# filodb/FiloDB

Measured on NVIDIA H100. Metric: samples/s scanned+aggregated (rate over 10M series); % HBM roofline, higher is better.
Workload: dtype f64

## Files before the change

### filodb_b200/csrc/scan_kernels.cu

```cuda
#include <cuda_runtime.h>
#include <stdint.h>
#define FILO_DEV_ERR_TS_WIRE 1
#define FILO_DEV_ERR_VAL_WIRE 2
#define FILO_DEV_ERR_EMPTY 3
#define FILO_DEV_ERR_SCRATCH 4
#include "scan_device.cuh"
#include "kernels.h"
#include "scan_fast.cuh"
#include "scan_tile.cuh"
#include "scan_wp.cuh"
#include "scan_wp_ctr.cuh"

namespace filo {

__device__ __forceinline__ void report_error(int* d_err, int code, int64_t series) {
  if (atomicCAS(&d_err[0], 0, code) == 0) { d_err[1] = (int)(series & 0x7fffffff); d_err[2] = (int)(series >> 31); }
}

__device__ __forceinline__ int resolve_series(const uint8_t* rec, const QueryParams& q, uint8_t* scratch, uint32_t scratch_bytes,
                                              bool need_corrected, int lane, int& err, int64_t& rows_scanned, int64_t& bytes_scanned) {
  const RecordHeader* h = reinterpret_cast<const RecordHeader*>(rec);
  const ChunkEntry* E = reinterpret_cast<const ChunkEntry*>(rec + sizeof(RecordHeader));
  const int nch = (int)h->n_chunks;
  const int64_t t1 = q.start - q.window, t2 = q.end;
// ... 342 lines not shown
                   unsigned long long* d_counters, int* d_err,
                   const int64_t* __restrict__ list, const unsigned long long* __restrict__ list_count) {
  MomOnly<MOM, double*> pval2;
  if constexpr (MOM) pval2.v = pval + (size_t)n_items * q.T;
  if (list) n_items = (int64_t)*list_count;
  extern __shared__ __align__(128) uint8_t smem[];
  const int warp = threadIdx.x >> 5, lane = threadIdx.x & 31;
  const int64_t gw = (int64_t)blockIdx.x * FAST_WARPS + warp, nw = (int64_t)gridDim.x * FAST_WARPS;
  const uint32_t per_warp = WARP_HDR_BYTES + rec_cap + STAGE_BYTES + acc_bytes + scratch_bytes;
  uint8_t* base = smem + (size_t)warp * per_warp;
  WarpStage st{reinterpret_cast<uint64_t*>(base), base + WARP_HDR_BYTES, rec_cap, 0, false, arena, rec_off};
  double* stage = reinterpret_cast<double*>(base + WARP_HDR_BYTES + rec_cap);
  double* acc = reinterpret_cast<double*>(base + WARP_HDR_BYTES + rec_cap + STAGE_BYTES);
  MomOnly<MOM, double*> acc2;
  if constexpr (MOM) acc2.v = acc + q.T;
  uint32_t* cnt = reinterpret_cast<uint32_t*>(base + WARP_HDR_BYTES + rec_cap + STAGE_BYTES + (size_t)q.T * (MOM ? 16 : 8));
  uint8_t* scratch = base + WARP_HDR_BYTES + rec_cap + STAGE_BYTES + acc_bytes;
  if (lane == 0) { mbar_init(st.bar, 1); mbar_fence_init(); }
  __syncwarp();
  const double ident = agg_op == AGG_MIN ? __longlong_as_double(0x7ff0000000000000LL)
                     : agg_op == AGG_MAX ? __longlong_as_double(0xfff0000000000000LL) : 0.0;
  int64_t rows = 0, bytes = 0;
  int64_t it = gw;
  int64_t pos = 0, pend = 0;
  auto real_item = [&](int64_t x) -> int64_t { return list ? list[x] : x; };
  auto advance_item = [&]() { while (it < n_items) { const int64_t ri = real_item(it); pos = item_begin[ri]; pend = item_begin[ri + 1]; if (pos < pend) return true; it += nw; } return false; };
  bool have = advance_item();
  if (have) st.issue(order ? order[pos] : pos, lane);
  while (have) {
    for (int k = lane; k < q.T; k += 32) { acc[k] = ident; cnt[k] = 0; if constexpr (MOM) acc2.v[k] = 0.0; }
    __syncwarp();
    const int64_t my_item = real_item(it);
    while (true) {
      const int64_t i = order ? order[pos] : pos;
      int64_t npos = pos + 1, nit = it, npend = pend; bool nhave = true;
      if (npos >= pend) { nit = it + nw; nhave = false; while (nit < n_items) { const int64_t ri = real_item(nit); npos = item_begin[ri]; npend = item_begin[ri + 1]; if (npos < npend) { nhave = true; break; } nit += nw; } }
      const int64_t inext = nhave ? (order ? order[npos] : npos) : -1;
      const uint8_t* rec = st.acquire(i);
      int err;
      process_series<CLS>(rec, q, scratch, scratch_bytes, stage, lane, err, rows, bytes,
                     [&](int k, double v, bool valid) {
                       if (valid && v == v) {
                         double a = acc[k];
                         if (agg_op == AGG_MIN) a = a < v ? a : v;
                         else if (agg_op == AGG_MAX) a = a > v ? a : v;
                         else if (agg_op != AGG_COUNT) a += v;
                         acc[k] = a; cnt[k] += 1;
                         if constexpr (MOM) acc2.v[k] += v * v;
                       }
                     },
                     [&]() { if (inext >= 0) st.issue(inext, lane); });
      if (err) {
        if (lane == 0) report_error(d_err, err, i);
        __syncwarp();
        if (inext >= 0) st.issue(inext, lane);
      }
      __syncwarp();
      const bool same_item = nhave && nit == it;
      pos = npos; pend = npend; it = nit; have = nhave;
      if (!same_item) break;
    }
    double* pv = pval + (size_t)my_item * q.T; uint32_t* pc = pcnt + (size_t)my_item * q.T;
    for (int k = lane; k < q.T; k += 32) { pv[k] = acc[k]; pc[k] = cnt[k]; }
    if constexpr (MOM) { double* pv2 = pval2.v + (size_t)my_item * q.T; for (int k = lane; k < q.T; k += 32) pv2[k] = acc2.v[k]; }
    __syncwarp();
  }
  if (lane == 0 && (rows | bytes)) { atomicAdd(&d_counters[0], (unsigned long long)rows); atomicAdd(&d_counters[1], (unsigned long long)bytes); }
}

#ifndef FILO_CUSIM
#ifdef FILO_TILE_PROF
extern "C" int filo_debug_tile_prof(unsigned long long* out16, int reset) {
  cudaError_t e = cudaMemcpyFromSymbol(out16, g_tile_prof, sizeof(unsigned long long) * 16);
  if (e == cudaSuccess && reset) { unsigned long long z[16] = {}; e = cudaMemcpyToSymbol(g_tile_prof, z, sizeof z); }
  return (int)e;
}
#endif
#ifdef FILO_WP_PROF
extern "C" int filo_debug_wp_prof(unsigned long long* out32, int reset) {
  cudaError_t e = cudaMemcpyFromSymbol(out32, g_wp_prof, sizeof(unsigned long long) * 32);
  if (e == cudaSuccess && reset) { unsigned long long z[32] = {}; e = cudaMemcpyToSymbol(g_wp_prof, z, sizeof z); }
  return (int)e;
}
#endif
template <int CLS>
static cudaError_t launch_series_v2_cls(const ScanLaunch& L, double* out, uint32_t rec_cap, size_t smem) {
  cudaError_t e = cudaFuncSetAttribute(scan_series_kernel_v2<CLS>, cudaFuncAttributeMaxDynamicSharedMemorySize, (int)smem);
  if (e != cudaSuccess) return e;
  scan_series_kernel_v2<CLS><<<L.grid, FAST_WARPS * 32, smem, L.stream>>>(L.arena, L.rec_off, L.n_series, L.q, out, rec_cap, L.scratch_bytes,
                                                                           L.d_counters, L.d_err, L.list, L.list_count);
  return cudaGetLastError();
}
cudaError_t launch_scan_series_v2(const ScanLaunch& L, double* out, uint32_t rec_cap) {
  const size_t smem = (size_t)(WARP_HDR_BYTES + rec_cap + STAGE_BYTES + L.scratch_bytes) * FAST_WARPS;
  switch (fn_class_of(L.q.fn, L.q.cumulative, L.q.long_values)) {
    case CLASS_SUM: return launch_series_v2_cls<CLASS_SUM>(L, out, rec_cap, smem);
    case CLASS_MINMAX: return launch_series_v2_cls<CLASS_MINMAX>(L, out, rec_cap, smem);
    case CLASS_COUNTER: return launch_series_v2_cls<CLASS_COUNTER>(L, out, rec_cap, smem);
    default: return launch_series_v2_cls<CLASS_POINT>(L, out, rec_cap, smem);
  }
}
template <int CLS, bool MOM>
static cudaError_t launch_agg_v2_cls(const ScanLaunch& L, const int32_t* order, const int64_t* item_begin, int64_t n_items, int agg_op,
                                     double* pval, uint32_t* pcnt, uint32_t acc_bytes, uint32_t rec_cap, size_t smem) {
  cudaError_t e = cudaFuncSetAttribute(scan_agg_kernel_v2<CLS, MOM>, cudaFuncAttributeMaxDynamicSharedMemorySize, (int)smem);
  if (e != cudaSuccess) return e;
  scan_agg_kernel_v2<CLS, MOM><<<L.grid, FAST_WARPS * 32, smem, L.stream>>>(L.arena, L.rec_off, order, item_begin, n_items, L.q, agg_op, pval, pcnt,
                                                                             rec_cap, L.scratch_bytes, acc_bytes, L.d_counters, L.d_err, L.list, L.list_count);
  return cudaGetLastError();
}
template <bool MOM>
static cudaError_t launch_agg_v2_any(const ScanLaunch& L, const int32_t* order, const int64_t* item_begin, int64_t n_items, int agg_op,
                                     double* pval, uint32_t* pcnt, uint32_t acc_bytes, uint32_t rec_cap, size_t smem) {
  switch (fn_class_of(L.q.fn, L.q.cumulative, L.q.long_values)) {
    case CLASS_SUM: return launch_agg_v2_cls<CLASS_SUM, MOM>(L, order, item_begin, n_items, agg_op, pval, pcnt, acc_bytes, rec_cap, smem);
    case CLASS_MINMAX: return launch_agg_v2_cls<CLASS_MINMAX, MOM>(L, order, item_begin, n_items, agg_op, pval, pcnt, acc_bytes, rec_cap, smem);
    case CLASS_COUNTER: return launch_agg_v2_cls<CLASS_COUNTER, MOM>(L, order, item_begin, n_items, agg_op, pval, pcnt, acc_bytes, rec_cap, smem);
    default: return launch_agg_v2_cls<CLASS_POINT, MOM>(L, order, item_begin, n_items, agg_op, pval, pcnt, acc_bytes, rec_cap, smem);
  }
}
cudaError_t launch_scan_agg_v2(const ScanLaunch& L, const int32_t* order, const int64_t* item_begin, int64_t n_items, int agg_op,
                               double* pval, uint32_t* pcnt, uint32_t acc_bytes, uint32_t rec_cap, bool moments) {
  const size_t smem = (size_t)(WARP_HDR_BYTES + rec_cap + STAGE_BYTES + acc_bytes + L.scratch_bytes) * FAST_WARPS;
  return moments ? launch_agg_v2_any<true>(L, order, item_begin, n_items, agg_op, pval, pcnt, acc_bytes, rec_cap, smem)
                 : launch_agg_v2_any<false>(L, order, item_begin, n_items, agg_op, pval, pcnt, acc_bytes, rec_cap, smem);
}
struct TileAggArgs { const int32_t* order; const int64_t* item_begin; int64_t n_items; int agg_op; double* pval; uint32_t* pcnt; };
template <int FN, bool AGG, bool MOM>
static cudaError_t launch_tile_fn(const ScanLaunch& L, double* out, const TileSmem& T, int64_t* fallback_list, unsigned long long* fallback_count,
                                  const TileAggArgs& A) {
  cudaError_t e = cudaFuncSetAttribute(scan_tile_kernel<FN, AGG, MOM>, cudaFuncAttributeMaxDynamicSharedMemorySize, (int)T.total);
  if (e != cudaSuccess) return e;
  scan_tile_kernel<FN, AGG, MOM><<<L.grid, TILE_LAUNCH_THREADS, T.total, L.stream>>>(L.arena, L.rec_off, L.n_series, L.q, out, T, fallback_list, fallback_count,
      L.d_counters, L.d_err, A.order, A.item_begin, A.n_items, A.agg_op, A.pval, A.pcnt);
  return cudaGetLastError();
}
template <bool AGG, bool MOM = false>
static cudaError_t launch_tile_any(const ScanLaunch& L, double* out, const TileSmem& T, int64_t* fallback_list, unsigned long long* fallback_count,
                                   const TileAggArgs& A) {
  switch (L.q.fn) {
    case FN_RATE: return launch_tile_fn<FN_RATE, AGG, MOM>(L, out, T, fallback_list, fallback_count, A);
    case FN_AVG: return launch_tile_fn<FN_AVG, AGG, MOM>(L, out, T, fallback_list, fallback_count, A);
    case FN_COUNT: return launch_tile_fn<FN_COUNT, AGG, MOM>(L, out, T, fallback_list, fallback_count, A);
    default: return launch_tile_fn<FN_SUM, AGG, MOM>(L, out, T, fallback_list, fallback_count, A);
  }
}
cudaError_t launch_scan_tile(const ScanLaunch& L, double* out, const TileSmem& T, int64_t* fallback_list, unsigned long long* fallback_count) {
  return launch_tile_any<false>(L, out, T, fallback_list, fallback_count, TileAggArgs{nullptr, nullptr, 0, 0, nullptr, nullptr});
}
cudaError_t launch_scan_tile_agg(const ScanLaunch& L, const TileSmem& T, const int32_t* order, const int64_t* item_begin, int64_t n_items, int agg_op,
                                 double* pval, uint32_t* pcnt, int64_t* fallback_list, unsigned long long* fallback_count, bool moments) {
  const TileAggArgs A{order, item_begin, n_items, agg_op, pval, pcnt};
  return moments ? launch_tile_any<true, true>(L, nullptr, T, fallback_list, fallback_count, A)
                 : launch_tile_any<true>(L, nullptr, T, fallback_list, fallback_count, A);
}
template <int FN, int NW>
static cudaError_t launch_wp_nw(const ScanLaunch& L, double* out, const WpSmem& W, int64_t* fallback_list, unsigned long long* fallback_count) {
  const size_t smem = (size_t)W.per_warp * W.warps;
  cudaError_t e = cudaFuncSetAttribute(scan_wp_sum_kernel<FN, NW>, cudaFuncAttributeMaxDynamicSharedMemorySize, (int)smem);
  if (e != cudaSuccess) return e;
  scan_wp_sum_kernel<FN, NW><<<L.grid, W.warps * 32, smem, L.stream>>>(L.arena, L.rec_off, L.n_series, L.q, out, W, fallback_list, fallback_count, L.d_counters, L.d_err);
  return cudaGetLastError();
}
template <int FN>
static cudaError_t launch_wp_fn(const ScanLaunch& L, double* out, const WpSmem& W, int64_t* fallback_list, unsigned long long* fallback_count) {
  if (W.warps <= (uint32_t)WP_MAX_WARPS) return launch_wp_nw<FN, WP_MAX_WARPS>(L, out, W, fallback_list, fallback_count);
// ... 123 lines not shown
```

### filodb_b200/csrc/scan_wp_ctr.cuh

```cuda
#pragma once
#include "scan_wp.cuh"

namespace filo {

__device__ __forceinline__ double drops_cum(const TileDrops& D, int r) {
  const int n = D.n < TILE_MAXDROP ? D.n : TILE_MAXDROP;
  double cum = 0.0;
#pragma unroll
  for (int j = 0; j < TILE_MAXDROP; ++j) if (j < n && D.pos[j] <= r) cum = D.amt[j];
  return cum;
}

template <bool IS_COUNTER, bool IS_RATE>
__device__ __forceinline__ double extrapolated_rate_tile(int64_t windowStart, int64_t windowEnd, int32_t numSamples, int64_t t1, double v1,
                                                         int64_t t2, double v2, double fdiv, double frcp, int64_t step, const TileCtrTab* tab) {
  double durationToStart = div_invariant((double)(t1 - windowStart), 1000.0, 0.001);
  const double durationToEnd = div_invariant((double)(windowEnd - t2), 1000.0, 0.001);
  const int64_t si_ms = t2 - t1;
  const int m = numSamples - 1;
  double sampledInterval, extrapolationThreshold, half, rcpSI;
  if (m <= TILE_CTR_TABMAX && si_ms == (int64_t)m * step) {
    const TileCtrTab e = tab[m];
    sampledInterval = e.sI; extrapolationThreshold = e.thr; half = e.half; rcpSI = e.rcpSI;
  } else {
// ... 34 lines not shown
    if (ch.end_time < wStart) continue;
    if (c > 0 && !(K[c - 1].end_time < wEnd)) continue;
    int su = ch.s0 + k; if (su < 0) su = 0;
    int eu = ch.e0 + k; if (eu > ch.nrows - 1) eu = ch.nrows - 1;
    const double first = __longlong_as_double((long long)CD[c].first);
    if (FN != FN_DELTA && some) { if (first != first || first < corrLast) corr = corr + corrLast; }
    if (su <= eu) {
      const int64_t tS = ch.init + (int64_t)su * qstep, tE = ch.init + (int64_t)eu * qstep;
      const bool skip = FN != FN_DELTA && su == 0 && eu == 0 && first != first;
      if (!skip && (tS < loT || tE > hiT)) {
        numSamples += eu - su + 1;
        const bool drp = FN != FN_DELTA && ch.kc.dropped;
        if (tS < loT) { loT = tS; const double b = wp_ctr_value(V, ch, su, DR[c], drp); loV = (FN != FN_DELTA && some) ? b + corr : b; }
        if (tE > hiT) { hiT = tE; const double b = wp_ctr_value(V, ch, eu, DR[c], drp); hiV = (FN != FN_DELTA && some) ? b + corr : b; }
      }
    }
    if (FN != FN_DELTA) {
      if (ch.kc.dropped) {
        int idx = ch.nrows - 1; double lastValue = 0.0;
        do { lastValue = wp_row(V, ch, idx); idx -= 1; } while (lastValue != lastValue && idx >= 0);
        corrLast = nan0(lastValue); corr = (some ? corr : 0.0) + drops_cum(DR[c], ch.nrows - 1);
      }
      else { corrLast = wp_row(V, ch, ch.nrows - 1); corr = some ? corr : 0.0; }
    }
    some = true;
  }
  const int64_t cws = qinclusive ? wStart : wStart - 1;
  if (hiT > loT) return extrapolated_rate_tile<FN != FN_DELTA, FN == FN_RATE>(cws, wEnd, numSamples, loT, loV, hiT, hiV, fdiv, frcp, qstep, tab);
  return NaNv;
}

__device__ __forceinline__ int wp_irr_lower(const int32_t* TSR, const WpCtrChunk& ch, int64_t t) {
  const int64_t d64 = t - ch.init;
  if (d64 <= 0) return 0;
  const int32_t* p = TSR + ch.rowpos;
  const int nr = ch.nrows;
  if (d64 > (int64_t)p[nr - 1]) return nr;
  const int32_t d = (int32_t)d64;
  int g = (int)((float)d * __int_as_float(ch.kc.pad));
  if (g > nr - 1) g = nr - 1;
  while (g < nr && p[g] < d) ++g;
  while (g > 0 && p[g - 1] >= d) --g;
  return g;
}
template <int FN>
__device__ __forceinline__ double wp_eval_counter_irr(int n, const WpCtrChunk* K, const WpChunk* CD, const TileDrops* DR, const double* V, const int32_t* TSR,
                                                      int64_t qstep, int qinclusive, int64_t wStart, int64_t wEnd, double fdiv, double frcp, const TileCtrTab* tab) {
  const double NaNv = __longlong_as_double(0x7ff8000000000000LL);
  int32_t numSamples = 0; int64_t loT = INT64_MAX, hiT = 0; double loV = NaNv, hiV = NaNv;
  bool some = false; double corrLast = 0.0, corr = 0.0;
  for (int c = 0; c < n; ++c) {
    const WpCtrChunk& ch = K[c];
    if (ch.end_time < wStart) continue;
    if (c > 0 && !(K[c - 1].end_time < wEnd)) continue;
    const int su = wp_irr_lower(TSR, ch, wStart);
    int eu = wp_irr_lower(TSR, ch, wEnd + 1) - 1; if (eu > ch.nrows - 1) eu = ch.nrows - 1;
    const double first = __longlong_as_double((long long)CD[c].first);
    if (FN != FN_DELTA && some) { if (first != first || first < corrLast) corr = corr + corrLast; }
    if (su <= eu) {
      const int64_t tS = ch.init + (int64_t)TSR[ch.rowpos + su], tE = ch.init + (int64_t)TSR[ch.rowpos + eu];
      const bool skip = FN != FN_DELTA && su == 0 && eu == 0 && first != first;
      if (!skip && (tS < loT || tE > hiT)) {
        numSamples += eu - su + 1;
        const bool drp = FN != FN_DELTA && ch.kc.dropped;
        if (tS < loT) { loT = tS; const double b = wp_ctr_value(V, ch, su, DR[c], drp); loV = (FN != FN_DELTA && some) ? b + corr : b; }
        if (tE > hiT) { hiT = tE; const double b = wp_ctr_value(V, ch, eu, DR[c], drp); hiV = (FN != FN_DELTA && some) ? b + corr : b; }
      }
    }
    if (FN != FN_DELTA) {
      if (ch.kc.dropped) {
        int idx = ch.nrows - 1; double lastValue = 0.0;
        do { lastValue = wp_row(V, ch, idx); idx -= 1; } while (lastValue != lastValue && idx >= 0);
        corrLast = nan0(lastValue); corr = (some ? corr : 0.0) + drops_cum(DR[c], ch.nrows - 1);
      }
      else { corrLast = wp_row(V, ch, ch.nrows - 1); corr = some ? corr : 0.0; }
    }
    some = true;
  }
  const int64_t cws = qinclusive ? wStart : wStart - 1;
  if (hiT > loT) return extrapolated_rate_tile<FN != FN_DELTA, FN == FN_RATE>(cws, wEnd, numSamples, loT, loV, hiT, hiV, fdiv, frcp, qstep, tab);
  return NaNv;
}

#ifdef FILO_CUSIM
inline void wp_bump_u16(uint16_t* p) { *p = (uint16_t)(*p + 1); }
#else
static __device__ __noinline__ void wp_bump_u16(uint16_t* p) { *p = (uint16_t)(*p + 1); }
#endif
template <int FN>
__device__ __forceinline__ double wp_clamped_window(const double* V, const WpCtrChunk& ch, const TileDrops& D, bool drp, int kk, int64_t wEnd, int64_t cws, int64_t qstep,
                                                   double fdiv, double frcp, const TileCtrTab* tab) {
  int r1 = ch.s0 + kk; if (r1 < 0) r1 = 0;
  int r2 = ch.e0 + kk; if (r2 > ch.nrows - 1) r2 = ch.nrows - 1;
  if (!(r2 > r1)) return __longlong_as_double(0x7ff8000000000000LL);
  double v1 = wp_row(V, ch, r1), v2 = wp_row(V, ch, r2);
  if (drp) { v1 = nan0(v1) + drops_cum(D, r1); v2 = nan0(v2) + drops_cum(D, r2); }
  return extrapolated_rate_tile<FN != FN_DELTA, FN == FN_RATE>(cws, wEnd, r2 - r1 + 1, ch.init + (int64_t)r1 * qstep, v1, ch.init + (int64_t)r2 * qstep, v2,
                                                              fdiv, frcp, qstep, tab);
}

template <int FN, bool AGG, int NW, bool IRR = false, bool MOM = false>
__global__ void __launch_bounds__(NW * 32, 1)
scan_wp_ctr_kernel(const uint8_t* __restrict__ arena, const int64_t* __restrict__ rec_off, int64_t n_series, QueryParams q,
                   double* __restrict__ out, WpCtrSmem L, int64_t* __restrict__ fallback_list, unsigned long long* __restrict__ fallback_count,
                   unsigned long long* d_counters, int* d_err,
                   const int32_t* __restrict__ order, const int64_t* __restrict__ item_begin, int64_t n_items, int agg_op,
                   double* __restrict__ pval, uint32_t* __restrict__ pcnt) {
  extern __shared__ __align__(128) uint8_t smem[];
  const unsigned FULL = 0xffffffffu;
  const int lane = threadIdx.x & 31, warp = threadIdx.x >> 5;
  uint8_t* wb = smem + (size_t)warp * L.per_warp;
  uint64_t* bar = reinterpret_cast<uint64_t*>(wb);
  WpChunk* CD = reinterpret_cast<WpChunk*>(wb + WP_OFF_DESC);
  uint64_t* xtab = reinterpret_cast<uint64_t*>(wb + WP_OFF_J);
  TileDrops* DR = reinterpret_cast<TileDrops*>(wb + WP_OFF_DROPS);
  uint8_t* R = wb + WP_OFF_REC;
  double* V = reinterpret_cast<double*>(wb + L.vals);
  WpCtrChunk* KC = reinterpret_cast<WpCtrChunk*>(wb + L.kc);
  double* ACC = reinterpret_cast<double*>(wb + L.acc);
  MomOnly<MOM, double*> ACC2;
  if constexpr (MOM) ACC2.v = reinterpret_cast<double*>(wb + L.nbad + align_up((uint32_t)q.T * 2u, 16));
  uint16_t* NBAD = reinterpret_cast<uint16_t*>(wb + L.nbad);
  int32_t* TSR = reinterpret_cast<int32_t*>(wb + L.tsr);
  constexpr bool allow_irr = IRR;
  TileCtrTab* CTAB = reinterpret_cast<TileCtrTab*>(smem + L.tab);
  const int64_t nwarps = (int64_t)gridDim.x * (blockDim.x >> 5);
  const int64_t gw = (int64_t)blockIdx.x * (blockDim.x >> 5) + warp;
  if (lane == 0) { mbar_init(bar, 1); mbar_fence_init(); }
  if ((int)threadIdx.x <= TILE_CTR_TABMAX) {
    const int m = threadIdx.x;
    TileCtrTab& e = CTAB[m];
    const double sI = (double)((int64_t)m * q.step) / 1000.0;
    const double avg = sI / ((double)(m + 1) - 1.0);
    e.sI = sI; e.thr = avg * 1.1; e.half = avg / 2.0; e.rcpSI = m > 0 ? 1.0 / sI : 0.0;
  }
  __syncthreads();

  int64_t winDur = q.inclusive ? q.window : q.window - 1; if (winDur < 0) winDur = 0;
  const double fdiv = (double)(q.inclusive ? winDur : winDur + 1), frcp = 1.0 / fdiv;
  const int64_t S0 = q.start - winDur, E0 = q.start;
  const int64_t lastEnd = q.start + (int64_t)(q.T - 1) * q.step;
  StepDiv sd; sd.init(q.step);
  const double NaNv = __longlong_as_double(0x7ff8000000000000LL);
  const double agg_ident = agg_op == AGG_MIN ? __longlong_as_double(0x7ff0000000000000LL)
                         : agg_op == AGG_MAX ? __longlong_as_double(0xfff0000000000000LL) : 0.0;

  int64_t m_init = 0, m_end = 0; int m_nrows = -1, m_n = -1, m_wire = -1, m_tlen = -1; bool m_ok = false;
  int dd_dst[2] = {0, 0}, dd_inf[2] = {0, 0};
  int64_t rows_scanned = 0, bytes_scanned = 0, pend_rows = 0, pend_bytes = 0;
  uint32_t parity = 0;

  int64_t c_it = 0, c_p = 0, c_pe = 0, x_it = 0, x_p = 0, x_pe = 0;
#define WP_ITEM_SEEK(it, p, pe, ok) { ok = false; while (it < n_items) { p = item_begin[it]; pe = item_begin[it + 1]; if (p < pe) { ok = true; break; } it += nwarps; } }
#define WP_POS_NEXT(it, p, pe, skip_item, ok) { \
    if (AGG) { if (!(skip_item) && p + 1 < pe) { p += 1; ok = true; } else { it += nwarps; WP_ITEM_SEEK(it, p, pe, ok) } } \
    else { p += nwarps; ok = p < n_series; } }
  auto sid_at = [&](int64_t p) -> int64_t { return (AGG && order) ? (int64_t)order[p] : p; };
  auto issue = [&](int64_t off, uint32_t sz) { mbar_expect_tx(bar, sz); tma_load_1d(R, arena + off, sz, bar); };

  bool more;
  if (AGG) { c_it = gw; WP_ITEM_SEEK(c_it, c_p, c_pe, more) } else { c_p = gw; c_pe = n_series; more = c_p < n_series; }
  int64_t cur_sid = 0, cur_off = 0; uint32_t cur_sz = 0;
  if (more) { cur_sid = sid_at(c_p); cur_off = rec_off[cur_sid]; cur_sz = (uint32_t)(rec_off[cur_sid + 1] - cur_off); }
  if (more && cur_sz <= L.rec_cap && lane == 0) issue(cur_off, cur_sz);
  bool item_bad = false; int item_nser = 0;
  if (AGG) { for (int k = lane; k < q.T; k += 32) { ACC[k] = agg_ident; NBAD[k] = 0; if constexpr (MOM) ACC2.v[k] = 0.0; } __syncwarp(); }

  while (more) {
    x_it = c_it; x_p = c_p; x_pe = c_pe; bool nmore;
    WP_POS_NEXT(x_it, x_p, x_pe, false, nmore)
    int64_t nxt_sid = 0, nxt_off = 0; uint32_t nxt_sz = 0;
    if (nmore) { nxt_sid = sid_at(x_p); nxt_off = rec_off[nxt_sid]; nxt_sz = (uint32_t)(rec_off[nxt_sid + 1] - nxt_off); }
    const bool staged = cur_sz <= L.rec_cap;
    if (staged) { mbar_wait(bar, parity); parity ^= 1; }
    const int64_t s = cur_sid;
    const bool skip = AGG && item_bad;
    const WpParsed P = wp_parse<false, IRR>(R, q, staged && !skip, lane);
    bool regular = P.regular;
    const bool irr = IRR && P.irr;
    const bool have = P.have; const int n = P.n, c = lane;
    const bool samec = !(c < n) || (P.init == m_init && P.nrows == m_nrows && P.end_time == m_end && P.vwire == m_wire && P.tlen == m_tlen);
    const bool same_all = __all_sync(FULL, samec);
    const bool same = m_ok && n == m_n && same_all && !irr;
    if (regular && !same) {
      m_init = P.init; m_end = P.end_time; m_nrows = P.nrows; m_n = n; m_wire = P.vwire; m_tlen = P.tlen; m_ok = false;
      const int64_t init = P.init, end_time = P.end_time; const int nrows = P.nrows, tlen = P.tlen;
      int64_t s0 = 0, e0 = 0, v4 = 0;
      if (have && !irr) { s0 = sd.ceil_div(S0 - init); e0 = sd.floor_div(E0 - init); v4 = sd.floor_div(end_time - S0); }
      const int64_t s0p = __shfl_up_sync(FULL, s0, 1), v4p = __shfl_up_sync(FULL, v4, 1), e0n = __shfl_down_sync(FULL, e0, 1);
      const int tlenp = __shfl_up_sync(FULL, tlen, 1);
      int64_t kA = -e0;
      if (c > 0) { int64_t x = v4p + 1; const int64_t y = (int64_t)tlenp - s0p; if (y > x) x = y; if (x > kA) kA = x; }
      int64_t kB = (int64_t)(nrows - 1) - s0;
      { const int64_t x = (c + 1 < n) ? -(e0n + 1) : (int64_t)q.T; if (x < kB) kB = x; }
      if (v4 < kB) kB = v4;
      if (kA < 0) kA = 0;
      if (kB > q.T - 1) kB = q.T - 1;
      const int64_t kA2 = kA, kB2 = kB;
      if (-s0 > kA) kA = -s0;
      { const int64_t x = (int64_t)(nrows - 1) - e0; if (x < kB) kB = x; }
      const int64_t sA = s0 + kA, eA = e0 + kA;
      const bool ok = have && !irr && kA <= kB && eA >= sA;
      const int Wr = ok ? (int)(eA - sA) : 0;
      const bool blocked = ok && Wr >= 1;
      int rowpos;
      { const int z = have ? nrows + 8 : 0;
        const int a0 = __shfl_sync(FULL, z, 0), a1 = __shfl_sync(FULL, z, 1), a2 = __shfl_sync(FULL, z, 2), a3 = __shfl_sync(FULL, z, 3);
        rowpos = (c > 0 ? a0 : 0) + (c > 1 ? a1 : 0) + (c > 2 ? a2 : 0);
        const int pend = a0 + a1 + a2 + a3;
        if ((uint32_t)(pend + (pend >> 3) + 2) > L.vcap) regular = false; }
      if (regular) {
        if (c < WP_MAXC) {
          WpCtrChunk& d = KC[c];
          d.init = init; d.end_time = end_time; d.nrows = nrows; d.s0 = (int)s0; d.e0 = (int)e0; d.rowpos = rowpos;
          d.kA = blocked ? (int)kA : 0; d.kB = blocked ? (int)kB : -1;
          d.kA2 = (have && !irr && kA2 <= kB2) ? (int)kA2 : 0; d.kB2 = (have && !irr && kA2 <= kB2) ? (int)kB2 : -1;
          if (irr) d.kc.pad = __float_as_int(have ? 1.0f / (float)P.tslope : 0.0f);
          if (blocked) {
            const double dTS = (double)(init + s0 * q.step - S0 + (q.inclusive ? 0 : 1)) / 1000.0, dTE = (double)(E0 - (init + e0 * q.step)) / 1000.0;
            const double sI = (double)((e0 - s0) * q.step) / 1000.0;
            const double avg = sI / ((double)(Wr + 1) - 1.0), thr = avg * 1.1, half = avg / 2.0;
            const double endpart = dTE < thr ? dTE : half;
            const double eTI = (sI + (dTS < thr ? dTS : half)) + endpart;
            d.kc.dTS = dTS; d.kc.thr = thr; d.kc.half = half; d.kc.endpart = endpart; d.kc.sI = sI; d.kc.ratio0 = eTI / sI;
            d.kc.skipC = 2.0 * dTS / sI;
          }
          CD[c].rowpos = rowpos; CD[c].nrows = nrows;
        }
        __syncwarp();
        {
          const int gb1 = __shfl_sync(FULL, have ? P.grp_base : 0x7fffffff, 1), gb2 = __shfl_sync(FULL, have ? P.grp_base : 0x7fffffff, 2),
                    gb3 = __shfl_sync(FULL, have ? P.grp_base : 0x7fffffff, 3);
#pragma unroll
          for (int jj = 0; jj < 2; ++jj) {
            const int slot = jj * 32 + lane;
            const bool active = slot < P.ngroups;
            const int ci = active ? (slot >= gb1 ? 1 : 0) + (slot >= gb2 ? 1 : 0) + (slot >= gb3 ? 1 : 0) : 0;
            const int gbc = ci == 0 ? 0 : ci == 1 ? gb1 : ci == 2 ? gb2 : gb3;
            const int g = active ? slot - gbc : 0;
            const int pq = CD[ci].rowpos + 1 + g * 8;
            dd_dst[jj] = wp_vidx(pq);
            dd_inf[jj] = (active ? 1 : 0) | (ci << 1) | ((pq & 7) << 3) | (g << 8);
          }
        }
        m_ok = !irr;
      }
    }
    bool declined = !regular && !skip;
    if (regular) {
      if (c < WP_MAXC) {
        WpChunk& d = CD[c];
        d.grp_base = have ? P.grp_base : 0x7fffffff; d.ng = P.ng; d.wire = P.vwire; d.val_off = P.voff; d.dropped = have ? P.dropped : 0;
        if (have && P.vwire == WIRE_XOR) { const uint32_t po = P.w12 >> 16; d.first = ld64(R + P.voff + po); d.grp_off = P.voff + po + 8; d.tab_off = P.voff + XOR_OFF_GROUPTAB; }
        else { d.first = have ? ld64(R + P.voff + 8) : 0ull; d.grp_off = 0; d.tab_off = 0; }
        KC[c].kc.dropped = have ? P.dropped : 0;
        DR[c].n = 0;
      }
      __syncwarp();
      (void)wp_decode<FN != FN_DELTA>(R, V, CD, xtab, dd_dst, dd_inf, n, P.any_raw, lane, DR);
      if (IRR && irr) {
        for (int ci = 0; ci < n; ++ci) {
          const uint32_t toff = __shfl_sync(FULL, P.toff, ci); const int tsl = __shfl_sync(FULL, P.tslope, ci);
          const uint8_t* tv = R + toff;
          const int nr = KC[ci].nrows; int32_t* dst = TSR + KC[ci].rowpos;
          if ((int)(ld32(tv + 4) & 0xffff) == WIRE_DDV) {
            const uint8_t* in = tv + 20; const uint32_t iw = ld32(in + 4);
            const int nbits = (iw >> 16) & 0x7f; const bool sgn = (iw >> 23) & 1;
            for (int r = lane; r < nr; r += 32) dst[r] = tsl * r + int_apply(in, nbits, sgn, r);
          } else for (int r = lane; r < nr; r += 32) dst[r] = tsl * r;
        }
      }
      __syncwarp();
      bool overflow = false;
      if (FN != FN_DELTA) for (int ci = 0; ci < n; ++ci) overflow |= KC[ci].kc.dropped && DR[ci].n > TILE_MAXDROP;
      if (overflow) { regular = false; declined = true; }
    }
    if (AGG && (declined || item_bad) && !skip) {
      x_it = c_it; x_p = c_p; x_pe = c_pe;
      WP_POS_NEXT(x_it, x_p, x_pe, true, nmore)
      if (nmore) { nxt_sid = sid_at(x_p); nxt_off = rec_off[nxt_sid]; nxt_sz = (uint32_t)(rec_off[nxt_sid + 1] - nxt_off); }
    }
    __syncwarp();
    if (nmore && nxt_sz <= L.rec_cap && lane == 0) issue(nxt_off, nxt_sz);

    if (declined) {
      if (!AGG) { if (lane == 0) { const unsigned long long slot = atomicAdd(fallback_count, 1ull); fallback_list[slot] = s; } }
      else item_bad = true;
    }
    if (regular && !skip) {
      int cnt_rows = 0, cnt_bytes = 0;
      { const int64_t endp = __shfl_up_sync(FULL, P.end_time, 1);
        if (have && !(c > 0 && !(endp < lastEnd))) { cnt_rows = P.num_rows; cnt_bytes = P.vbytes; } }
#pragma unroll
      for (int o = 1; o < WP_MAXC; o <<= 1) { cnt_rows += __shfl_xor_sync(FULL, cnt_rows, o); cnt_bytes += __shfl_xor_sync(FULL, cnt_bytes, o); }
      if (lane == 0) { pend_rows += cnt_rows; pend_bytes += cnt_bytes; }
      if (FN != FN_DELTA && lane < n && KC[lane].kc.dropped) {
        TileDrops& D = DR[lane];
        const int nd = D.n;
        for (int i = 1; i < nd; ++i) {
          const int pz = D.pos[i]; const double a = D.amt[i]; int j = i - 1;
          while (j >= 0 && D.pos[j] > pz) { D.pos[j + 1] = D.pos[j]; D.amt[j + 1] = D.amt[j]; --j; }
          D.pos[j + 1] = pz; D.amt[j + 1] = a;
        }
        double run = 0.0;
        for (int i = 0; i < nd; ++i) { run += D.amt[i]; D.amt[i] = run; }
      }
      __syncwarp();
      double* gout = AGG ? nullptr : out + (size_t)s * q.T;
      const bool agg_add = agg_op == AGG_SUM || agg_op == AGG_AVG;
      auto emit = [&](int k, double v) {
        if (!AGG) { wp_store_result(gout + k, v); return; }
        if (v == v) {
          if (agg_add) ACC[k] += v;
          else if (agg_op != AGG_COUNT) { const double a = ACC[k]; if (agg_op == AGG_MIN ? !(a < v) : !(a > v)) ACC[k] = v; }
          if constexpr (MOM) ACC2.v[k] += v * v;
        } else wp_bump_u16(NBAD + k);
      };
      for (int ci = 0; ci < n; ++ci) {
        const WpCtrChunk& ch = KC[ci];
        if (ch.kA2 > ch.kB2) continue;
        const bool hasfast = ch.kA <= ch.kB;
        const TileCtr kc = ch.kc;
        const TileDrops& D = DR[ci];
        const bool drp = FN != FN_DELTA && kc.dropped;
        const int dn = drp ? D.n : 0;
        const int dpos0 = dn >= 1 ? D.pos[0] : 0x7fffffff;
        const double damt0 = dn >= 1 ? D.amt[0] : 0.0;
        const double* p1 = V + wp_vidx(ch.rowpos + ch.s0 + ch.kA + lane);
        const double* p2 = V + wp_vidx(ch.rowpos + ch.e0 + ch.kA + lane);
        auto fast_one = [&](int kk, double v1, double v2) -> double {
          if (drp) {
            const int r1 = ch.s0 + kk, r2 = ch.e0 + kk;
            if (dn <= 1) { v1 = nan0(v1) + (r1 >= dpos0 ? damt0 : 0.0); v2 = nan0(v2) + (r2 >= dpos0 ? damt0 : 0.0); }
            else { v1 = nan0(v1) + drops_cum(D, r1); v2 = nan0(v2) + drops_cum(D, r2); }
          }
          const double delta = v2 - v1;
          double ratio = kc.ratio0;
          if (FN != FN_DELTA && delta > 0 && v1 >= 0 && !(v1 > delta * kc.skipC)) {
            const double dz = kc.sI * ddiv_rare(v1, delta);
            const double dts = dz < kc.dTS ? dz : kc.dTS;
            const double eTI = (kc.sI + (dts < kc.thr ? dts : kc.half)) + kc.endpart;
            ratio = ddiv_rare(eTI, kc.sI);
          }
          const double scaled = delta * ratio;
          return FN == FN_RATE ? __dmul_rn(div_invariant(scaled, fdiv, frcp), 1000.0) : scaled;
        };
#ifdef FILO_WP_CTR_PAIR
        for (int kk = ch.kA + lane; hasfast && kk <= ch.kB; kk += 64, p1 += 72, p2 += 72) {
          const bool two = kk + 32 <= ch.kB;
          const double a1 = *p1, a2 = *p2;
          const double b1 = two ? p1[36] : 0.0, b2 = two ? p2[36] : 0.0;
          const double ra = fast_one(kk, a1, a2);
          const double rb = two ? fast_one(kk + 32, b1, b2) : 0.0;
          emit(kk, ra);
          if (two) emit(kk + 32, rb);
        }
#else
        for (int kk = ch.kA + lane; hasfast && kk <= ch.kB; kk += 32, p1 += 36, p2 += 36) emit(kk, fast_one(kk, *p1, *p2));
#endif
        const int nlo = hasfast ? ch.kA - ch.kA2 : ch.kB2 - ch.kA2 + 1, nhi = hasfast ? ch.kB2 - ch.kB : 0;
        for (int u = lane; u < nlo + nhi; u += 32) {
          const int kk = u < nlo ? ch.kA2 + u : ch.kB + 1 + (u - nlo);
          const int64_t wEnd = q.start + (int64_t)kk * q.step, cws = wEnd - winDur - (q.inclusive ? 0 : 1);
          emit(kk, wp_clamped_window<FN>(V, ch, D, drp, kk, wEnd, cws, q.step, fdiv, frcp, CTAB));
        }
      }
      {
        int prev = -1;
        for (int ci = 0; ci <= n; ++ci) {
          int gend = q.T;
          if (ci < n) { if (KC[ci].kA2 > KC[ci].kB2) continue; gend = KC[ci].kA2; }
          for (int k = prev + 1 + lane; k < gend; k += 32) {
            const int64_t wEnd = q.start + (int64_t)k * q.step, wStart = wEnd - winDur;
            if (IRR && irr) emit(k, wp_eval_counter_irr<FN>(n, KC, CD, DR, V, TSR, q.step, q.inclusive, wStart, wEnd, fdiv, frcp, CTAB));
            else emit(k, wp_eval_counter<FN>(n, KC, CD, DR, V, q.step, q.inclusive, wStart, wEnd, k, fdiv, frcp, CTAB));
          }
          if (ci < n) prev = KC[ci].kB2;
        }
      }
      if (!AGG && lane == 0) { rows_scanned += pend_rows; bytes_scanned += pend_bytes; pend_rows = 0; pend_bytes = 0; }
      if (AGG) item_nser += 1;
    }
    if (AGG) {
      const bool last_of_item = !nmore || x_it != c_it;
      if (last_of_item) {
        __syncwarp();
        if (!item_bad) {
          double* pv = pval + (size_t)c_it * q.T; uint32_t* pc = pcnt + (size_t)c_it * q.T;
          for (int k = lane; k < q.T; k += 32) { pv[k] = ACC[k]; pc[k] = (uint32_t)(item_nser - (int)NBAD[k]); }
          if constexpr (MOM) { double* pv2 = pval + (size_t)(n_items + c_it) * q.T; for (int k = lane; k < q.T; k += 32) pv2[k] = ACC2.v[k]; }
          if (lane == 0) { rows_scanned += pend_rows; bytes_scanned += pend_bytes; }
        } else if (lane == 0) {
          const unsigned long long slot = atomicAdd(fallback_count, 1ull); fallback_list[slot] = c_it;
        }
        for (int k = lane; k < q.T; k += 32) { ACC[k] = agg_ident; NBAD[k] = 0; if constexpr (MOM) ACC2.v[k] = 0.0; }
        pend_rows = 0; pend_bytes = 0; item_bad = false; item_nser = 0;
      }
    }
    __syncwarp();
    c_it = x_it; c_p = x_p; c_pe = x_pe; more = nmore; cur_sid = nxt_sid; cur_off = nxt_off; cur_sz = nxt_sz;
  }
  if (lane == 0 && (rows_scanned | bytes_scanned)) {
    atomicAdd(&d_counters[0], (unsigned long long)rows_scanned); atomicAdd(&d_counters[1], (unsigned long long)bytes_scanned);
  }
}

#undef WP_ITEM_SEEK
#undef WP_POS_NEXT

}
```

### filodb_b200/csrc/scan_wp_layout.h

```cpp
#pragma once
#include <stdint.h>
#include "filo_record.h"
#include "scan_params.h"
#include "scan_tile_layout.h"
namespace filo {
constexpr int WP_MAXC = 4;
constexpr int WP_MAXG = 64;
constexpr int WP_R = 8;
constexpr int WP_MAX_WARPS = 16;
constexpr int WP_MAX_WARPS_ALIAS = 20;

struct WpChunk {
  uint64_t first;
  int32_t kT0, kT1;
  int32_t ownLo, ownHi;
  int32_t blk0, nblk;
  int32_t vidx0;
  int32_t rowpos;
  int32_t nrows, s0, e0;
  int32_t grp_base, ng, wire;
  uint32_t grp_off, tab_off, val_off;
  int32_t joff, hs;
  int32_t jzb, tb;
  int32_t dropped;
// ... 29 lines not shown
  L.per_warp = align_up(o, 16);
  L.warps = 0;
  L.alias = alias ? 1u : 0u;
  return L;
}

constexpr int WP_BATCH_WARPS = 16;
constexpr int WP_BATCH_SERIES = 15;
constexpr int WP_BATCH_BUFS = 2;
struct WpEntryChunk {
  uint64_t first;
  int64_t init, end_time;
  uint32_t grp_off, val_off;
  int32_t nrows, grp_base, ng;
  uint32_t wire;
};
static_assert(sizeof(WpEntryChunk) == 48, "WpEntryChunk");
struct WpEntry {
  uint32_t rofs;
  int32_t n;
  int32_t flags;
  int32_t ngroups, cnt_rows, cnt_bytes;
  int32_t pad[2];
  WpEntryChunk c[WP_MAXC];
};
static_assert(sizeof(WpEntry) == 224, "WpEntry");
struct WpBatchSmem {
  WpSmem W;
  uint32_t B, nbuf, consumers;
  uint32_t buf, buf_stride, buf_cap;
  uint32_t ent;
  uint32_t bars;
  uint32_t total;
  uint32_t rt, rtcap;
};
FILO_HD inline WpBatchSmem wp_batch_layout(uint32_t max_rec_bytes, uint32_t max_rows, uint32_t max_chunks, uint32_t T, uint32_t wrows, bool alias,
                                           uint32_t B = WP_BATCH_SERIES, uint32_t nbuf = WP_BATCH_BUFS, uint32_t consumers = WP_BATCH_WARPS - 1) {
  WpBatchSmem S;
  WpSmem L = wp_layout(max_rec_bytes, max_rows, max_chunks, T, wrows, alias);
  const uint32_t shift = L.vals - WP_OFF_REC;
  L.vals -= shift; L.out -= shift; L.per_warp -= shift; L.rec = 0;
  const uint32_t mc = max_chunks < (uint32_t)WP_MAXC ? max_chunks : (uint32_t)WP_MAXC;
  S.rtcap = mc > 1 ? (uint32_t)WP_R * (mc - 1) * ((wrows + 14) / 8) : 0;
  S.rt = L.out + 8 * (T + 1);
  { const uint32_t oreg = alias ? L.vcap : L.ocap, need = T + 1 + S.rtcap;
    L.per_warp = align_up(L.out + 8 * (oreg > need ? oreg : need), 16); }
  S.consumers = consumers;
  L.warps = S.consumers;
  S.W = L; S.B = B; S.nbuf = nbuf;
  uint32_t o = L.per_warp * S.consumers;
  S.buf = o;
  S.buf_cap = B * align_up(max_rec_bytes, 16);
  S.buf_stride = S.buf_cap + 16;
  o += nbuf * S.buf_stride;
  S.ent = o; o += nbuf * B * (uint32_t)sizeof(WpEntry);
  S.bars = o; o += 3 * nbuf * 8;
  S.total = align_up(o, 16);
  return S;
}

FILO_HD inline uint32_t wp_max_items(uint32_t max_chunks, uint32_t T, uint32_t wrows) {
  if (max_chunks > (uint32_t)WP_MAXC) max_chunks = WP_MAXC;
  if (max_chunks == 0) max_chunks = 1;
  return (T + (max_chunks - 1) * (wrows - 1) + 7 * max_chunks) / 8;
}

constexpr int WP_CTR_MAX_WARPS = 20;
struct TileCtr {
  double dTS, thr, half, endpart, sI, ratio0, skipC;
  int32_t dropped, pad;
};
constexpr int TILE_MAXDROP = 8;
constexpr int TILE_CTR_TABMAX = 64;
struct TileCtrTab { double sI, thr, half, rcpSI; };
struct TileDrops {
  int32_t n, pos[TILE_MAXDROP], pad[3];
  double amt[TILE_MAXDROP];
};
struct WpCtrChunk {
  int64_t init, end_time;
  int32_t nrows, s0, e0, rowpos;
  int32_t kA, kB;
  int32_t kA2, kB2;
  TileCtr kc;
};
static_assert(sizeof(WpCtrChunk) == 112, "WpCtrChunk");

struct WpCtrSmem {
  uint32_t vals, kc, acc, nbad, per_warp, tab ;
  uint32_t rec_cap, vcap , warps, agg;
  uint32_t tsr;
};
constexpr uint32_t WP_OFF_DROPS = WP_OFF_J + 64 * 8;
static_assert(WP_OFF_DROPS + WP_MAXC * sizeof(TileDrops) <= WP_OFF_REC, "drops fit in front of the record");
FILO_HD inline WpCtrSmem wp_ctr_layout(uint32_t max_rec_bytes, uint32_t max_rows, uint32_t max_chunks, uint32_t T, bool agg, bool irr = false,
                                       bool moments = false) {
  WpCtrSmem L;
  if (max_chunks > (uint32_t)WP_MAXC) max_chunks = WP_MAXC;
  L.rec_cap = align_up(max_rec_bytes + 16, 16);
  const uint32_t P = max_rows + 8 * max_chunks + 8;
  L.vcap = align_up(P + P / 8 + 2, 2);
  uint32_t o = WP_OFF_REC + L.rec_cap;
  L.vals = o; o += L.vcap * 8;
  L.kc = o; o += (uint32_t)(WP_MAXC * sizeof(WpCtrChunk));
  L.tsr = 0;
  if (irr) { L.tsr = o; o += align_up(P * 4, 16); }
  L.acc = o; L.nbad = o;
  if (agg) { o += T * 8; L.nbad = o; o += align_up(T * 2, 16); }
  if (agg && moments) o += T * 8;
  L.per_warp = align_up(o, 16);
  L.tab = 0; L.warps = 0; L.agg = agg ? 1u : 0u;
  return L;
}
FILO_HD inline bool wp_ctr_tile_footprint_ok(uint32_t max_rec_bytes, uint32_t max_rows, uint32_t T, uint64_t cap) {
  const uint32_t ctr = 2 * align_up(TILE_NS * TILE_MAXC * (uint32_t)sizeof(TileCtr), 128) + align_up(TILE_NS * TILE_MAXC * (uint32_t)sizeof(TileDrops), 128) +
                       align_up((TILE_CTR_TABMAX + 1) * (uint32_t)sizeof(TileCtrTab), 128);
  return (uint64_t)(tile_layout(max_rec_bytes, max_rows, T, 0).total + ctr) + 1024 <= cap;
}

enum { SCAN_PATH_V2 = 0, SCAN_PATH_TILE = 1, SCAN_PATH_WP_SUM = 2, SCAN_PATH_WP_BATCH = 3, SCAN_PATH_WP_CTR = 4 };
struct ScanPathIn {
  uint32_t max_rec_bytes, max_rows, max_chunks, T;
  uint64_t wrows;
  int fn_cls;
  bool fused, moments;
  bool irr;
  bool v2;
  int force;
  uint64_t smem_cap;
  int64_t n_series;
  int64_t n_items;
  int sm_count;
};
struct ScanPath {
  int kernel;
  bool tile, wp, wp_batch, wp_ctr;
  bool refused;
  int tile_ctas_per_sm;
  int grid;
  int fused_kernel;
  int fused_grid;
  TileSmem TL; WpSmem WL; WpBatchSmem WB; WpCtrSmem WC;
};
FILO_HD inline ScanPath scan_path(const ScanPathIn& in) {
  ScanPath P{};
  P.kernel = SCAN_PATH_V2;
  const uint32_t T = in.T, wrows = (uint32_t)in.wrows;
  if (in.v2 && in.force != 2 && in.fn_cls == CLASS_SUM && in.n_series > 0) {
    P.TL = tile_layout(in.max_rec_bytes, in.max_rows, T, (uint32_t)(2 * in.wrows < (1u << 20) ? 2 * in.wrows : (1u << 20)) + 16);
    if (((uint64_t)P.TL.total + 1024) * 2 > (uint64_t)228 * 1024) P.TL = tile_layout(in.max_rec_bytes, in.max_rows, T, 16);
    P.tile = (uint64_t)P.TL.total + 1024 <= in.smem_cap;
  }
  P.tile_ctas_per_sm = ((uint64_t)P.TL.total + 1024) * 2 <= (uint64_t)228 * 1024 ? 2 : 1;
  if (P.tile && in.force != 3 && in.wrows <= 4096 && in.max_chunks > 0) {
    const bool alias = wp_max_items(in.max_chunks, T, wrows) <= 64;
    P.WL = wp_layout(in.max_rec_bytes, in.max_rows, in.max_chunks, T, wrows, alias);
    { const uint64_t w = in.smem_cap / P.WL.per_warp, wmax = alias ? WP_MAX_WARPS_ALIAS : WP_MAX_WARPS; P.WL.warps = (uint32_t)(w < wmax ? w : wmax); }
    const WpSmem WL2 = wp_layout(in.max_rec_bytes, in.max_rows, in.max_chunks, T, wrows, alias, true);
    if (in.smem_cap / WL2.per_warp >= (uint64_t)WP_MAX_WARPS) {
      P.WL = WL2; P.WL.warps = WP_MAX_WARPS;
      P.WB = wp_batch_layout(in.max_rec_bytes, in.max_rows, in.max_chunks, T, wrows, alias);
      P.wp_batch = P.WB.total <= in.smem_cap;
      if (P.wp_batch && P.WB.W.alias && wp_max_items(in.max_chunks, T, wrows) > 64) P.refused = true;
    }
    P.wp = P.WL.warps >= 4;
  }
  if (in.v2 && in.force != 2 && in.force != 3 && in.fn_cls == CLASS_COUNTER && in.n_series > 0 && in.max_chunks > 0 &&
      (!in.fused || T <= (uint32_t)(TILE_AGG_ACC * TILE_THREADS)) && wp_ctr_tile_footprint_ok(in.max_rec_bytes, in.max_rows, T, in.smem_cap)) {
    P.WC = wp_ctr_layout(in.max_rec_bytes, in.max_rows, in.max_chunks, T, in.fused, in.irr, in.moments);
// ... 23 lines not shown
```

Before: 173.4 billion.

## Add fast path for counter windows spanning two adjacent chunks

Per series, the kernel now computes a junction range [jA, jB] for each pair of contiguous regular chunks. Windows in that range, which start in one chunk and end in the next, are evaluated directly from two row values plus a reset correction through a shared helper (wp_ctr_fast). Before, each such window went through the general per-window wp_eval_counter walk over all chunks; the gap-fold loop now skips windows already handled. The cost is more descriptor setup (extra warp shuffles and a larger WpCtrChunk) and a per-window membership check in the gap loop. Clock-based phase profiling macros and a host readout script are also added, compiled only under FILO_WP_PROF.

New measurement: 173.5 billion, median of 6. No clear change (+0.0%).

```diff
diff --git a/filodb_b200/csrc/scan_kernels.cu b/filodb_b200/csrc/scan_kernels.cu
--- a/filodb_b200/csrc/scan_kernels.cu
+++ b/filodb_b200/csrc/scan_kernels.cu
@@ -448,6 +448,11 @@
   if (e == cudaSuccess && reset) { unsigned long long z[32] = {}; e = cudaMemcpyToSymbol(g_wp_prof, z, sizeof z); }
   return (int)e;
 }
+extern "C" int filo_debug_ctr_prof(unsigned long long* out16, int reset) {
+  cudaError_t e = cudaMemcpyFromSymbol(out16, g_ctr_prof, sizeof(unsigned long long) * 16);
+  if (e == cudaSuccess && reset) { unsigned long long z[16] = {}; e = cudaMemcpyToSymbol(g_ctr_prof, z, sizeof z); }
+  return (int)e;
+}
 #endif
 template <int CLS>
 static cudaError_t launch_series_v2_cls(const ScanLaunch& L, double* out, uint32_t rec_cap, size_t smem) {
diff --git a/filodb_b200/csrc/scan_wp_ctr.cuh b/filodb_b200/csrc/scan_wp_ctr.cuh
--- a/filodb_b200/csrc/scan_wp_ctr.cuh
+++ b/filodb_b200/csrc/scan_wp_ctr.cuh
@@ -140,6 +140,20 @@
   return NaNv;
 }
 
+template <int FN>
+__device__ __forceinline__ double wp_ctr_fast(const TileCtr& kc, double v1, double v2, double fdiv, double frcp) {
+  const double delta = v2 - v1;
+  double ratio = kc.ratio0;
+  if (FN != FN_DELTA && delta > 0 && v1 >= 0 && !(v1 > delta * kc.skipC)) {
+    const double dz = kc.sI * ddiv_rare(v1, delta);
+    const double dts = dz < kc.dTS ? dz : kc.dTS;
+    const double eTI = (kc.sI + (dts < kc.thr ? dts : kc.half)) + kc.endpart;
+    ratio = ddiv_rare(eTI, kc.sI);
+  }
+  const double scaled = delta * ratio;
+  return FN == FN_RATE ? __dmul_rn(div_invariant(scaled, fdiv, frcp), 1000.0) : scaled;
+}
+
 #ifdef FILO_CUSIM
 inline void wp_bump_u16(uint16_t* p) { *p = (uint16_t)(*p + 1); }
 #else
@@ -156,6 +170,19 @@
   return extrapolated_rate_tile<FN != FN_DELTA, FN == FN_RATE>(cws, wEnd, r2 - r1 + 1, ch.init + (int64_t)r1 * qstep, v1, ch.init + (int64_t)r2 * qstep, v2,
                                                               fdiv, frcp, qstep, tab);
 }
+
+#if defined(FILO_WP_PROF) && !defined(FILO_CUSIM)
+__device__ unsigned long long g_ctr_prof[16];
+#define CPROF_DECL uint32_t cpp_t0 = (uint32_t)clock(), cpp_acc[14] = {0, 0, 0, 0, 0, 0, 0, 0, 0, 0, 0, 0, 0, 0};
+#define CPROF(i) { const uint32_t cpp_t1 = (uint32_t)clock(); cpp_acc[i] += cpp_t1 - cpp_t0; cpp_t0 = cpp_t1; }
+#define CPROF_COUNT(i) { ++cpp_acc[i]; }
+#define CPROF_FLUSH if (lane == 0) { for (int cpp_i = 0; cpp_i < 14; ++cpp_i) atomicAdd(&g_ctr_prof[cpp_i], (unsigned long long)cpp_acc[cpp_i]); atomicAdd(&g_ctr_prof[15], 1ull); }
+#else
+#define CPROF_DECL
+#define CPROF(i)
+#define CPROF_COUNT(i)
+#define CPROF_FLUSH
+#endif
 
 template <int FN, bool AGG, int NW, bool IRR = false, bool MOM = false>
 __global__ void __launch_bounds__(NW * 32, 1)
@@ -223,6 +250,7 @@
   if (more && cur_sz <= L.rec_cap && lane == 0) issue(cur_off, cur_sz);
   bool item_bad = false; int item_nser = 0;
   if (AGG) { for (int k = lane; k < q.T; k += 32) { ACC[k] = agg_ident; NBAD[k] = 0; if constexpr (MOM) ACC2.v[k] = 0.0; } __syncwarp(); }
+  CPROF_DECL
 
   while (more) {
     x_it = c_it; x_p = c_p; x_pe = c_pe; bool nmore;
@@ -230,10 +258,14 @@
     int64_t nxt_sid = 0, nxt_off = 0; uint32_t nxt_sz = 0;
     if (nmore) { nxt_sid = sid_at(x_p); nxt_off = rec_off[nxt_sid]; nxt_sz = (uint32_t)(rec_off[nxt_sid + 1] - nxt_off); }
     const bool staged = cur_sz <= L.rec_cap;
+    CPROF(10)
     if (staged) { mbar_wait(bar, parity); parity ^= 1; }
+    CPROF(0)
+    CPROF_COUNT(11)
     const int64_t s = cur_sid;
     const bool skip = AGG && item_bad;
     const WpParsed P = wp_parse<false, IRR>(R, q, staged && !skip, lane);
+    CPROF(1)
     bool regular = P.regular;
     const bool irr = IRR && P.irr;
     const bool have = P.have; const int n = P.n, c = lane;
@@ -241,6 +273,7 @@
     const bool same_all = __all_sync(FULL, samec);
     const bool same = m_ok && n == m_n && same_all && !irr;
     if (regular && !same) {
+      CPROF_COUNT(12)
       m_init = P.init; m_end = P.end_time; m_nrows = P.nrows; m_n = n; m_wire = P.vwire; m_tlen = P.tlen; m_ok = false;
       const int64_t init = P.init, end_time = P.end_time; const int nrows = P.nrows, tlen = P.tlen;
       int64_t s0 = 0, e0 = 0, v4 = 0;
@@ -261,6 +294,26 @@
       const bool ok = have && !irr && kA <= kB && eA >= sA;
       const int Wr = ok ? (int)(eA - sA) : 0;
       const bool blocked = ok && Wr >= 1;
+      int64_t jA = 0, jB = -1;
+      { const int64_t initn = __shfl_down_sync(FULL, init, 1), s0n = __shfl_down_sync(FULL, s0, 1), v4n = __shfl_down_sync(FULL, v4, 1);
+        const int64_t endn = __shfl_down_sync(FULL, end_time, 1);
+        const int nrowsn = __shfl_down_sync(FULL, nrows, 1);
+        const bool blockedn = __shfl_down_sync(FULL, blocked, 1);
+        if (!IRR && have && c + 1 < n && nrows >= 2 && initn == init + (int64_t)nrows * q.step && (blocked || blockedn)) {
+          jA = 0;
+          if (-s0 > jA) jA = -s0;
+          if ((int64_t)(nrows - 1) - e0 > jA) jA = (int64_t)(nrows - 1) - e0;
+          if (-e0n > jA) jA = -e0n;
+          if (c > 0 && v4p + 1 > jA) jA = v4p + 1;
+          { const int64_t x = sd.floor_div(end_time - E0) + 1; if (x > jA) jA = x; }
+          jB = q.T - 1;
+          if (v4 < jB) jB = v4;
+          if ((int64_t)(nrows - 1) - s0 < jB) jB = (int64_t)(nrows - 1) - s0;
+          if (-s0n < jB) jB = -s0n;
+          if ((int64_t)(nrowsn - 1) - e0n < jB) jB = (int64_t)(nrowsn - 1) - e0n;
+          if (v4n < jB) jB = v4n;
+          if (c + 2 < n) { const int64_t x = sd.floor_div(endn - E0); if (x < jB) jB = x; }
+        } }
       int rowpos;
       { const int z = have ? nrows + 8 : 0;
         const int a0 = __shfl_sync(FULL, z, 0), a1 = __shfl_sync(FULL, z, 1), a2 = __shfl_sync(FULL, z, 2), a3 = __shfl_sync(FULL, z, 3);
@@ -273,6 +326,7 @@
           d.init = init; d.end_time = end_time; d.nrows = nrows; d.s0 = (int)s0; d.e0 = (int)e0; d.rowpos = rowpos;
           d.kA = blocked ? (int)kA : 0; d.kB = blocked ? (int)kB : -1;
           d.kA2 = (have && !irr && kA2 <= kB2) ? (int)kA2 : 0; d.kB2 = (have && !irr && kA2 <= kB2) ? (int)kB2 : -1;
+          d.jA = jA <= jB ? (int)jA : 0; d.jB = jA <= jB ? (int)jB : -1;
           if (irr) d.kc.pad = __float_as_int(have ? 1.0f / (float)P.tslope : 0.0f);
           if (blocked) {
             const double dTS = (double)(init + s0 * q.step - S0 + (q.inclusive ? 0 : 1)) / 1000.0, dTE = (double)(E0 - (init + e0 * q.step)) / 1000.0;
@@ -304,6 +358,7 @@
         m_ok = !irr;
       }
     }
+    CPROF(2)
     bool declined = !regular && !skip;
     if (regular) {
       if (c < WP_MAXC) {
@@ -315,6 +370,7 @@
         DR[c].n = 0;
       }
       __syncwarp();
+      CPROF(3)
       (void)wp_decode<FN != FN_DELTA>(R, V, CD, xtab, dd_dst, dd_inf, n, P.any_raw, lane, DR);
       if (IRR && irr) {
         for (int ci = 0; ci < n; ++ci) {
@@ -340,8 +396,10 @@
     }
     __syncwarp();
     if (nmore && nxt_sz <= L.rec_cap && lane == 0) issue(nxt_off, nxt_sz);
+    CPROF(4)
 
     if (declined) {
+      CPROF_COUNT(13)
       if (!AGG) { if (lane == 0) { const unsigned long long slot = atomicAdd(fallback_count, 1ull); fallback_list[slot] = s; } }
       else item_bad = true;
     }
@@ -364,6 +422,7 @@
         for (int i = 0; i < nd; ++i) { run += D.amt[i]; D.amt[i] = run; }
       }
       __syncwarp();
+      CPROF(5)
       double* gout = AGG ? nullptr : out + (size_t)s * q.T;
       const bool agg_add = agg_op == AGG_SUM || agg_op == AGG_AVG;
       auto emit = [&](int k, double v) {
@@ -392,16 +451,7 @@
             if (dn <= 1) { v1 = nan0(v1) + (r1 >= dpos0 ? damt0 : 0.0); v2 = nan0(v2) + (r2 >= dpos0 ? damt0 : 0.0); }
             else { v1 = nan0(v1) + drops_cum(D, r1); v2 = nan0(v2) + drops_cum(D, r2); }
           }
-          const double delta = v2 - v1;
-          double ratio = kc.ratio0;
-          if (FN != FN_DELTA && delta > 0 && v1 >= 0 && !(v1 > delta * kc.skipC)) {
-            const double dz = kc.sI * ddiv_rare(v1, delta);
-            const double dts = dz < kc.dTS ? dz : kc.dTS;
-            const double eTI = (kc.sI + (dts < kc.thr ? dts : kc.half)) + kc.endpart;
-            ratio = ddiv_rare(eTI, kc.sI);
-          }
-          const double scaled = delta * ratio;
-          return FN == FN_RATE ? __dmul_rn(div_invariant(scaled, fdiv, frcp), 1000.0) : scaled;
+          return wp_ctr_fast<FN>(kc, v1, v2, fdiv, frcp);
         };
 #ifdef FILO_WP_CTR_PAIR
         for (int kk = ch.kA + lane; hasfast && kk <= ch.kB; kk += 64, p1 += 72, p2 += 72) {
@@ -416,11 +466,40 @@
 #else
         for (int kk = ch.kA + lane; hasfast && kk <= ch.kB; kk += 32, p1 += 36, p2 += 36) emit(kk, fast_one(kk, *p1, *p2));
 #endif
+        CPROF(6)
         const int nlo = hasfast ? ch.kA - ch.kA2 : ch.kB2 - ch.kA2 + 1, nhi = hasfast ? ch.kB2 - ch.kB : 0;
         for (int u = lane; u < nlo + nhi; u += 32) {
           const int kk = u < nlo ? ch.kA2 + u : ch.kB + 1 + (u - nlo);
           const int64_t wEnd = q.start + (int64_t)kk * q.step, cws = wEnd - winDur - (q.inclusive ? 0 : 1);
           emit(kk, wp_clamped_window<FN>(V, ch, D, drp, kk, wEnd, cws, q.step, fdiv, frcp, CTAB));
+        }
+        CPROF(7)
+      }
+      unsigned jfast = 0;
+      for (int ci = 0; !IRR && ci + 1 < n; ++ci) {
+        const WpCtrChunk& ch = KC[ci];
+        if (ch.jA > ch.jB) continue;
+        const double first = __longlong_as_double((long long)CD[ci + 1].first);
+        if (first != first) continue;
+        jfast |= 1u << ci;
+        const WpCtrChunk& nx = KC[ci + 1];
+        double corr = 0.0;
+        if (FN != FN_DELTA) {
+          double corrLast;
+          if (ch.kc.dropped) {
+            int idx = ch.nrows - 1; double lastValue = 0.0;
+            do { lastValue = wp_row(V, ch, idx); idx -= 1; } while (lastValue != lastValue && idx >= 0);
+            corrLast = nan0(lastValue); corr = 0.0 + drops_cum(DR[ci], ch.nrows - 1);
+          }
+          else { corrLast = wp_row(V, ch, ch.nrows - 1); corr = 0.0; }
+          if (first != first || first < corrLast) corr = corr + corrLast;
+        }
+        const TileCtr& kt = ch.kA <= ch.kB ? ch.kc : nx.kc;
+        const bool drp1 = FN != FN_DELTA && ch.kc.dropped, drp2 = FN != FN_DELTA && nx.kc.dropped;
+        for (int k = ch.jA + lane; k <= ch.jB; k += 32) {
+          const double v1 = wp_ctr_value(V, ch, ch.s0 + k, DR[ci], drp1);
+          const double b = wp_ctr_value(V, nx, nx.e0 + k, DR[ci + 1], drp2);
+          emit(k, wp_ctr_fast<FN>(kt, v1, FN != FN_DELTA ? b + corr : b, fdiv, frcp));
         }
       }
       {
@@ -429,6 +508,9 @@
           int gend = q.T;
           if (ci < n) { if (KC[ci].kA2 > KC[ci].kB2) continue; gend = KC[ci].kA2; }
           for (int k = prev + 1 + lane; k < gend; k += 32) {
+            bool done = false;
+            for (int j = 0; !IRR && j + 1 < n; ++j) done |= ((jfast >> j) & 1u) && k >= KC[j].jA && k <= KC[j].jB;
+            if (done) continue;
             const int64_t wEnd = q.start + (int64_t)k * q.step, wStart = wEnd - winDur;
             if (IRR && irr) emit(k, wp_eval_counter_irr<FN>(n, KC, CD, DR, V, TSR, q.step, q.inclusive, wStart, wEnd, fdiv, frcp, CTAB));
             else emit(k, wp_eval_counter<FN>(n, KC, CD, DR, V, q.step, q.inclusive, wStart, wEnd, k, fdiv, frcp, CTAB));
@@ -436,6 +518,7 @@
           if (ci < n) prev = KC[ci].kB2;
         }
       }
+      CPROF(8)
       if (!AGG && lane == 0) { rows_scanned += pend_rows; bytes_scanned += pend_bytes; pend_rows = 0; pend_bytes = 0; }
       if (AGG) item_nser += 1;
     }
@@ -454,6 +537,7 @@
         for (int k = lane; k < q.T; k += 32) { ACC[k] = agg_ident; NBAD[k] = 0; if constexpr (MOM) ACC2.v[k] = 0.0; }
         pend_rows = 0; pend_bytes = 0; item_bad = false; item_nser = 0;
       }
+      CPROF(9)
     }
     __syncwarp();
     c_it = x_it; c_p = x_p; c_pe = x_pe; more = nmore; cur_sid = nxt_sid; cur_off = nxt_off; cur_sz = nxt_sz;
@@ -461,6 +545,7 @@
   if (lane == 0 && (rows_scanned | bytes_scanned)) {
     atomicAdd(&d_counters[0], (unsigned long long)rows_scanned); atomicAdd(&d_counters[1], (unsigned long long)bytes_scanned);
   }
+  CPROF_FLUSH
 }
 
 #undef WP_ITEM_SEEK
diff --git a/filodb_b200/csrc/scan_wp_layout.h b/filodb_b200/csrc/scan_wp_layout.h
--- a/filodb_b200/csrc/scan_wp_layout.h
+++ b/filodb_b200/csrc/scan_wp_layout.h
@@ -135,9 +135,10 @@
   int32_t nrows, s0, e0, rowpos;
   int32_t kA, kB;
   int32_t kA2, kB2;
+  int32_t jA, jB;
   TileCtr kc;
 };
-static_assert(sizeof(WpCtrChunk) == 112, "WpCtrChunk");
+static_assert(sizeof(WpCtrChunk) == 120, "WpCtrChunk");
 
 struct WpCtrSmem {
   uint32_t vals, kc, acc, nbad, per_warp, tab ;
diff --git a/scratch/ctr_prof.py b/scratch/ctr_prof.py
--- /dev/null
+++ b/scratch/ctr_prof.py
@@ -0,0 +1,32 @@
+import ctypes as C
+import os
+import sys
+
+import numpy as np
+
+HERE = os.path.dirname(os.path.abspath(__file__))
+sys.path.insert(0, os.path.dirname(HERE))
+import filodb_b200.capi as capi
+capi.LIB_PATH = os.environ.get("FILO_LIB_PATH") or os.path.join(HERE, "libfilo_b200_wp_prof.so")
+import bench
+
+workload = sys.argv[1] if len(sys.argv) > 1 else "c5"
+series = sys.argv[2] if len(sys.argv) > 2 else "5000000"
+L = capi.lib()
+L.filo_debug_ctr_prof.argtypes = [C.c_void_p, C.c_int]
+out = np.zeros(16, np.uint64)
+sys.argv = ["bench.py", "--workload", workload, "--series", series, "--steps", "4", "--warmup", "2", "--no-e2e", "--no-cpu", "--no-extra", "--no-c5"]
+L.filo_debug_ctr_prof(out.ctypes.data, 1)
+bench.main()
+L.filo_debug_ctr_prof(out.ctypes.data, 0)
+names = ["wait: record (mbarrier)", "parse", "memo check (+ window plan on a miss)", "per-series descriptors", "decode (+ next copy issued)",
+         "scan counters, drop sort", "fast windows + emit", "clamped windows + emit", "junction and gap fold + emit", "item flush",
+         "loop head, declined series"]
+ns = float(out[11])
+tot = float(out[:11].sum())
+print("%s: counter kernel, %d warps, %d series taken up, %d memo misses, %d declined"
+      % (workload, int(out[15]), int(ns), int(out[12]), int(out[13])))
+print("  %-40s %10s %7s" % ("phase", "cyc/series", "share"))
+for i, n in enumerate(names):
+    print("  %-40s %10.1f %6.1f %%" % (n, float(out[i]) / ns, 100.0 * float(out[i]) / tot))
+print("  %-40s %10.1f" % ("total", tot / ns))
```
